# Eric-Canas/Homography.js

Measured on AMD Instinct MI355X. Metric: Mpixels/s warped (piecewise-affine, 4K RGBA), higher is better.
Workload: dtype u8 pixels / f64 coordinates

## Files before the change

### homography.js_amd/csrc/hg_api_piecewise.hip

```cpp
#include "hg_ctx.h"

extern "C" int hg_piecewise_set_mesh(hg_ctx *c, const float *src, int n_pts, const uint32_t *tris, int n_tris, int msx, int msy)
{
    HG_TRY(bind(c));
    if (!src || n_pts <= 0 || n_tris < 0 || (!tris && n_tris > 0)) return fail(c, HG_ERR_INVALID, "hg_piecewise_set_mesh: bad arguments");
    if (!coords_ok(src, (size_t)n_pts * 2))
        return fail(c, HG_ERR_INVALID, "hg_piecewise_set_mesh: a source coordinate is infinite or beyond 2^24 in magnitude");
    if (c->have_mesh && n_pts == c->n_pts && n_tris == c->n_tris && msx == c->min_src_x && msy == c->min_src_y &&
        std::memcmp(src, c->h_src.data(), sizeof(float) * 2 * (size_t)n_pts) == 0 &&
        (n_tris == 0 || std::memcmp(tris, c->h_tris.data(), sizeof(uint32_t) * 3 * (size_t)n_tris) == 0))
        return HG_OK;
    HG_TRY(hg_sync(c));
    HG_TRY(ensure(c, c->d_src, (size_t)n_pts * 2));
    HG_TRY(ensure(c, c->d_tris, (size_t)std::max(n_tris, 1) * 3));
    HIP_TRY(c, hipMemcpyAsync(c->d_src, src, sizeof(float) * 2 * n_pts, hipMemcpyHostToDevice, c->stream));
    if (n_tris > 0) HIP_TRY(c, hipMemcpyAsync(c->d_tris, tris, sizeof(uint32_t) * 3 * n_tris, hipMemcpyHostToDevice, c->stream));
    HIP_TRY(c, hipStreamSynchronize(c->stream));
    c->n_pts = n_pts; c->n_tris = n_tris; c->min_src_x = msx; c->min_src_y = msy;
    c->h_tris.assign(tris, tris + (size_t)3 * n_tris);
    c->h_src.assign(src, src + (size_t)2 * n_pts);
    c->fmap_valid = false;
    c->have_mesh = true;
    c->mesh_gen++; c->pw_epoch++;
    c->fwd_pw_tiles_disabled = false; c->fwd_pw_cap = 64;
// ... 407 lines not shown
    c->status_next = c->status_base + (size_t)((c->status_slot + 1) % (int)kStatusRing) * F;
    c->rows_clean = false;
    if (p.self) {
        c->pw_gen = c->pw_gen >= 0x7ffffff0 ? 1 : c->pw_gen + 1;
        launch_tri_setup(mesh_of(c), frames_of(c), c->stream);
    } else launch_tri_spans(mesh_of(c), frames_of(c), rl, c->stream);
    HIP_TRY(c, hipGetLastError());
    c->pw_setup_done = true;
    return HG_OK;
}

static SpanPlanKey span_key_of(const hg_ctx *c)
{
    const PwPlan &p = c->pw_plan;
    SpanPlanKey k;
    k.eligible = p.kernel == PwKernel::Rows && p.self && p.row_group == kRowGroup && c->n_imgs <= 1;
    k.W = c->W; k.H = c->H;
    if (c->pw_moving) { k.ms_lo_x = c->ms_lo_x; k.ms_hi_x = c->ms_hi_x; k.ms_lo_y = c->ms_lo_y; k.ms_hi_y = c->ms_hi_y; }
    else { k.ms_lo_x = k.ms_hi_x = c->min_src_x; k.ms_lo_y = k.ms_hi_y = c->min_src_y; }
    k.hi_bounds = p.no_hi_bounds ? 0 : 1;
    k.safe_spans = p.safe_spans; k.bands = p.bands ? 1 : 0; k.n_bands = p.n_bands;
    k.n_frames = (int)c->pw_frames.size(); k.max_h = c->pw_shape.max_h;
    return k;
}

static int span_cache_prepare(hg_ctx *c, SpanCacheDev *sc)
{
    *sc = SpanCacheDev();
    c->span_last = 0;
    if (c->opt_span_cache == 0) return HG_OK;
    const SpanPlanKey key = span_key_of(c);
    if (!key.eligible) return HG_OK;
    const PwShape &s = c->pw_shape;
    const uint64_t estimate = (uint64_t)s.groups * kRowGroup * (uint64_t)std::min(s.cover + 1, 63) * (kSpanRecWordsLong * 16);
    const bool force = c->opt_span_cache_mb < 0;
    const uint64_t budget = force ? (uint64_t)(-(int64_t)c->opt_span_cache_mb) << 10 : (uint64_t)c->opt_span_cache_mb << 20;
    const SpanCacheMode mode = span_cache_decide(c->span_state, c->pw_epoch, key, c->opt_span_cache, budget, estimate, force);
    if (mode == SpanCacheMode::Build) {
        const uint64_t bytes = std::min<uint64_t>(force ? budget : std::min(budget, estimate), ((uint64_t)1 << 36) - 16);
        const int gpf = (std::max(s.max_h, 1) + kRowGroup - 1) / kRowGroup;
        const size_t entries = 1 + (size_t)key.n_frames * gpf;
        HG_TRY(ensure(c, c->d_span_rec, (size_t)std::max<uint64_t>(bytes / 16, 1)));
        HG_TRY(ensure(c, c->d_span_dir, entries));
        HIP_TRY(c, hipMemsetAsync(c->d_span_dir, 0, sizeof(int4) * entries, c->stream));
        c->span_cap16 = (uint32_t)(bytes / 16); c->span_gpf = gpf;
        c->span_builds++;
    }
    span_cache_commit(c->span_state, c->pw_epoch, key, c->opt_span_cache, mode);
    if (mode == SpanCacheMode::Off) return HG_OK;
    if (mode == SpanCacheMode::Use) c->span_uses++;
    c->span_last = (int)mode;
    sc->dir = c->d_span_dir + 1; sc->rec = c->d_span_rec; sc->cursor = reinterpret_cast<unsigned long long *>(c->d_span_dir.p);
    sc->cap16 = c->span_cap16; sc->groups_per_frame = c->span_gpf; sc->mode = (int)mode;
    return HG_OK;
}

extern "C" int hg_span_cache_stats(hg_ctx *c, int64_t out[6])
{
    HG_TRY(bind(c));
    if (!out) return fail(c, HG_ERR_INVALID, "hg_span_cache_stats: out is NULL");
    out[0] = c->span_builds; out[1] = c->span_uses; out[2] = 0; out[3] = 0; out[4] = 0; out[5] = c->span_last;
    const SpanCacheState &st = c->span_state;
    if (!st.built || st.epoch != c->pw_epoch || !c->d_span_dir.cap || (size_t)st.key.n_frames != c->pw_frames.size()) return HG_OK;
    const size_t entries = 1 + (size_t)st.key.n_frames * c->span_gpf;
    std::vector<int4> dir(entries);
    HIP_TRY(c, hipStreamSynchronize(c->stream));
    HIP_TRY(c, hipMemcpy(dir.data(), c->d_span_dir, sizeof(int4) * entries, hipMemcpyDeviceToHost));
    for (size_t f = 0; f < c->pw_frames.size(); f++) {
        const FrameDesc &fd = c->pw_frames[f];
        if (fd.obj_w <= 0 || fd.obj_h <= 0) continue;
        for (int g = 0; g < (fd.obj_h + kRowGroup - 1) / kRowGroup; g++) {
            const int32_t state = dir[1 + f * (size_t)c->span_gpf + g].x;
// ... 364 lines not shown
```

### homography.js_amd/csrc/hg_dev.h

```cpp
#pragma once
#include "hg_kernels.h"
#include <cstdlib>
#include <type_traits>

namespace hg {

__device__ __forceinline__ void flag_frame(const PwFrames &fr, int f, int32_t bits)
{
    atomicOr(&fr.status[f], bits);
    if (fr.host_flag) __hip_atomic_store(fr.host_flag, 1, __ATOMIC_RELAXED, __HIP_MEMORY_SCOPE_SYSTEM);
}



extern "C" __device__ uint32_t hg_struct_load_u32(__amdgpu_buffer_rsrc_t rsrc, int vindex, int voffset, int soffset, int aux) __asm("llvm.amdgcn.struct.ptr.buffer.load.i32");

__device__ __forceinline__ bool frame_group(const PwFrames &fr, int xcd, int bi, int groups_per_xcd, int &f, int &g)
{
    if (fr.sub_groups > 0) {
        const int per_sub = fr.sub_groups * fr.n_frames, sb = bi / per_sub, rem = bi - sb * per_sub;
        f = rem / fr.sub_groups;
        g = ((sb << fr.xcc_log2) + xcd) * fr.sub_groups + (rem - f * fr.sub_groups);
        return g < (groups_per_xcd << fr.xcc_log2);
    }
    f = bi / groups_per_xcd;
    g = ((xcd + (fr.xcc_rotate ? f : 0)) & ((1 << fr.xcc_log2) - 1)) * groups_per_xcd + (bi - f * groups_per_xcd);
    return true;
}
inline int sub_groups_of(const PwFrames &fr, int groups_per_xcd) { return fr.sub_bands > 1 ? (groups_per_xcd + fr.sub_bands - 1) / fr.sub_bands : 0; }
inline int padded_groups(int groups_per_xcd, int sub_groups) { return sub_groups > 0 ? ((groups_per_xcd + sub_groups - 1) / sub_groups) * sub_groups : groups_per_xcd; }

struct HiBounds { uint32_t lox, rx, loy, ry; };
__host__ __device__ __forceinline__ bool hi_bounds_ok(int64_t ax, int64_t bx, int64_t ay, int64_t by)
{
    return ax >= 0 && ay >= 0 && bx < (1 << 20) && by < (1 << 20) && ax <= bx && ay <= by;
}
inline bool set_hi_bounds_ok(const PwMesh &mesh, const PwFrames &fr)
{
    if (!fr.min_src) return hi_bounds_ok(mesh.min_src_x, (int64_t)mesh.W + mesh.min_src_x, mesh.min_src_y, (int64_t)mesh.H + mesh.min_src_y);
    return hi_bounds_ok(fr.min_src_lo_x, (int64_t)mesh.W + fr.min_src_hi_x, fr.min_src_lo_y, (int64_t)mesh.H + fr.min_src_hi_y);
}
__device__ __forceinline__ HiBounds make_hi_bounds(double lox, double hix, double loy, double hiy)
{
    HiBounds b;
    b.lox = (uint32_t)__builtin_amdgcn_readfirstlane(__double2hiint(lox)); b.rx = (uint32_t)__builtin_amdgcn_readfirstlane(__double2hiint(hix)) - b.lox;
    b.loy = (uint32_t)__builtin_amdgcn_readfirstlane(__double2hiint(loy)); b.ry = (uint32_t)__builtin_amdgcn_readfirstlane(__double2hiint(hiy)) - b.loy;
    return b;
}
__device__ __forceinline__ bool hi_inb(const HiBounds &b, double hx, double hy)
{
    return (int)(((uint32_t)__double2hiint(hx) - b.lox) < b.rx) & (int)(((uint32_t)__double2hiint(hy) - b.loy) < b.ry);
}

__device__ __forceinline__ int round_inbounds(double x)
{
    double r = floor(x);
    if (x - r >= 0.5) r += 1.0;
    return (int)r;
}

__device__ __forceinline__ int64_t floordiv64(int64_t n, int64_t d)
{
    int64_t q = n / d;
    if ((n % d) < 0) --q;
    return q;
}

__device__ __forceinline__ uint32_t fetch_src(const uint32_t *__restrict__ img32, int64_t n_src_px, int W, int rx, int ry)
{
    const int64_t idx = (int64_t)ry * W + rx;
    return (idx >= 0 && idx < n_src_px) ? img32[idx] : 0u;
}

__device__ __forceinline__ void store_quad(uint32_t *__restrict__ orow, int cq, int W, bool vec_ok, const uint32_t px[4])
{
    if (vec_ok && cq + 3 < W) {
        *reinterpret_cast<uint4 *>(orow + cq) = make_uint4(px[0], px[1], px[2], px[3]);
    } else {
#pragma unroll
// ... 79 lines not shown

__device__ __forceinline__ uint32_t pw_pixel_bilinear(int tid_raw, int x, double y, MatCache &mc, const float *__restrict__ invm,
                                                      const uint32_t *__restrict__ img32, int W, int H,
                                                      double bx0, double bx1, double by0, double by1)
{
    const int t16 = (int)(int16_t)tid_raw;
    if (t16 < 0) return 0u;
    if (t16 != mc.id) {
        const float4 lo = *reinterpret_cast<const float4 *>(invm + (size_t)t16 * kInvStride);
        const float2 hi = *reinterpret_cast<const float2 *>(invm + (size_t)t16 * kInvStride + 4);
        mc.m[0] = lo.x; mc.m[1] = lo.y; mc.m[2] = lo.z; mc.m[3] = lo.w; mc.m[4] = hi.x; mc.m[5] = hi.y;
        mc.id = t16;
    }
    const double xd = (double)x;
    const double sx = (mc.m[0] * xd) + (mc.m[2] * y) + mc.m[4];
    const double sy = (mc.m[1] * xd) + (mc.m[3] * y) + mc.m[5];
    if (sx >= bx0 && sx < bx1 && sy >= by0 && sy < by1) return bilinear_fetch(img32, W, H, sx, sy);
    return 0u;
}

template <int S>
__device__ __forceinline__ uint32_t pw_pixel_mode(int tid_raw, int x, double y, MatCache &mc, const float *__restrict__ invm,
                                                  const uint32_t *__restrict__ img32, int64_t n_src_px, int W, int H,
                                                  double bx0, double bx1, double by0, double by1)
{
    if (S == 1) return pw_pixel_bilinear(tid_raw, x, y, mc, invm, img32, W, H, bx0, bx1, by0, by1);
    return pw_pixel(tid_raw, x, y, mc, invm, img32, n_src_px, W, H, bx0, bx1, by0, by1);
}

__device__ __forceinline__ uint32_t dlo(double v) { return (uint32_t)__double2loint(v); }
__device__ __forceinline__ double sgpr_f64(double v)
{
    return __hiloint2double(__builtin_amdgcn_readfirstlane(__double2hiint(v)), __builtin_amdgcn_readfirstlane(__double2loint(v)));
}

constexpr int kStoreNT = 2;
constexpr int kKeyShift = 14, kKeyOffMask = (1 << kKeyShift) - 1;

__device__ __forceinline__ void round_x8(double h[8], double r[8])
{
    const double M = 6755399441055744.0;
    asm(
        "s_setreg_imm32_b32 hwreg(HW_REG_MODE, 2, 2), 2\n\t"
        "v_add_f64 %0, %0, 0.5\n\t"  "v_add_f64 %1, %1, 0.5\n\t"  "v_add_f64 %2, %2, 0.5\n\t"  "v_add_f64 %3, %3, 0.5\n\t"
        "v_add_f64 %4, %4, 0.5\n\t"  "v_add_f64 %5, %5, 0.5\n\t"  "v_add_f64 %6, %6, 0.5\n\t"  "v_add_f64 %7, %7, 0.5\n\t"
        "v_add_f64 %8, %0, %16\n\t"  "v_add_f64 %9, %1, %16\n\t"  "v_add_f64 %10, %2, %16\n\t" "v_add_f64 %11, %3, %16\n\t"
        "v_add_f64 %12, %4, %16\n\t" "v_add_f64 %13, %5, %16\n\t" "v_add_f64 %14, %6, %16\n\t" "v_add_f64 %15, %7, %16\n\t"
        "s_setreg_imm32_b32 hwreg(HW_REG_MODE, 2, 2), 0"
        : "+v"(h[0]), "+v"(h[1]), "+v"(h[2]), "+v"(h[3]), "+v"(h[4]), "+v"(h[5]), "+v"(h[6]), "+v"(h[7]),
          "=&v"(r[0]), "=&v"(r[1]), "=&v"(r[2]), "=&v"(r[3]), "=&v"(r[4]), "=&v"(r[5]), "=&v"(r[6]), "=&v"(r[7])
        : "s"(M));
}

__device__ __forceinline__ void round_x4(double h[4], double r[4])
{
    const double M = 6755399441055744.0;
    asm volatile(
        "s_setreg_imm32_b32 hwreg(HW_REG_MODE, 2, 2), 2\n\t"
        "v_add_f64 %0, %0, 0.5\n\t" "v_add_f64 %1, %1, 0.5\n\t" "v_add_f64 %2, %2, 0.5\n\t" "v_add_f64 %3, %3, 0.5\n\t"
        "v_add_f64 %4, %0, %8\n\t"  "v_add_f64 %5, %1, %8\n\t"  "v_add_f64 %6, %2, %8\n\t"  "v_add_f64 %7, %3, %8\n\t"
        "s_setreg_imm32_b32 hwreg(HW_REG_MODE, 2, 2), 0"
        : "+v"(h[0]), "+v"(h[1]), "+v"(h[2]), "+v"(h[3]), "=&v"(r[0]), "=&v"(r[1]), "=&v"(r[2]), "=&v"(r[3])
        : "s"(M));
}

__device__ __forceinline__ void round_half_x4(const double v[4], int r[4])
// ... 38 lines not shown
        : [d0] "v"(d), [d1] "v"(d1), [d2] "v"(d2), [d3] "v"(d3), [len] "v"(len), [key] "v"(key)
        : "vcc");
}

__device__ __forceinline__ void span_max4s(int best[4], int d, int len, int key)
{
    const int d1 = d + 64, d2 = d + 128, d3 = d + 192;
    unsigned long long sv;
    asm volatile(
        "s_mov_b64 %[sv], exec\n\t"
        "v_cmpx_gt_u32_e32 vcc, %[len], %[d0]\n\t" "v_max_i32_e32 %[b0], %[key], %[b0]\n\t" "s_mov_b64 exec, %[sv]\n\t"
        "v_cmpx_gt_u32_e32 vcc, %[len], %[d1]\n\t" "v_max_i32_e32 %[b1], %[key], %[b1]\n\t" "s_mov_b64 exec, %[sv]\n\t"
        "v_cmpx_gt_u32_e32 vcc, %[len], %[d2]\n\t" "v_max_i32_e32 %[b2], %[key], %[b2]\n\t" "s_mov_b64 exec, %[sv]\n\t"
        "v_cmpx_gt_u32_e32 vcc, %[len], %[d3]\n\t" "v_max_i32_e32 %[b3], %[key], %[b3]\n\t" "s_mov_b64 exec, %[sv]"
        : [b0] "+v"(best[0]), [b1] "+v"(best[1]), [b2] "+v"(best[2]), [b3] "+v"(best[3]), [sv] "=&s"(sv)
        : [d0] "v"(d), [d1] "v"(d1), [d2] "v"(d2), [d3] "v"(d3), [len] "s"(len), [key] "s"(key)
        : "vcc");
}

__device__ __forceinline__ void span_max4d(int best[4], int d0, int d1, int d2, int d3, int len, int key)
{
    unsigned long long sv;
    asm volatile(
        "s_mov_b64 %[sv], exec\n\t"
        "v_cmpx_lt_u32_e32 vcc, %[d0], %[len]\n\t" "v_max_i32_e32 %[b0], %[b0], %[key]\n\t" "s_mov_b64 exec, %[sv]\n\t"
        "v_cmpx_lt_u32_e32 vcc, %[d1], %[len]\n\t" "v_max_i32_e32 %[b1], %[b1], %[key]\n\t" "s_mov_b64 exec, %[sv]\n\t"
        "v_cmpx_lt_u32_e32 vcc, %[d2], %[len]\n\t" "v_max_i32_e32 %[b2], %[b2], %[key]\n\t" "s_mov_b64 exec, %[sv]\n\t"
        "v_cmpx_lt_u32_e32 vcc, %[d3], %[len]\n\t" "v_max_i32_e32 %[b3], %[b3], %[key]\n\t" "s_mov_b64 exec, %[sv]"
        : [b0] "+v"(best[0]), [b1] "+v"(best[1]), [b2] "+v"(best[2]), [b3] "+v"(best[3]), [sv] "=&s"(sv)
        : [d0] "v"(d0), [d1] "v"(d1), [d2] "v"(d2), [d3] "v"(d3), [len] "v"(len), [key] "v"(key)
        : "vcc");
}

}

#include "hg_spans.h"
```

### homography.js_amd/csrc/hg_k_piecewise.hip

```cpp
#include "hg_dev.h"
#include <type_traits>

namespace hg {

constexpr int kBandMax = 2048;

__device__ __forceinline__ bool tri_setup_one(const PwMesh &mesh, const PwFrames &fr, int f, int t, const FrameDesc &fd, TriRange &tr)
{
    float d[6], inv[6];
    Seg seg[3];
    tri_solve(mesh, fr, f, t, true, d, inv, seg);
    const size_t ft = (size_t)f * mesh.n_tris + t;
    const bool one_fma = affine_fusable(inv, coord_bits(fd.x_off, fd.obj_w), coord_bits(fd.y_off, fd.obj_h));

    tri_rows_tight(d[1], d[3], d[5], tr.y_min, tr.y_end);
    tr.a = 0; tr.b = 0;
    const bool too_tall = (tr.y_end - (int64_t)tr.y_min) > (1 << 24);
    {
        int64_t y_first = tr.y_min, y_stop = tr.y_end;
        if (fd.obj_w > 0 && fd.obj_h > 0) clamp_rows(y_first, y_stop, fd.y_off, fd.obj_w, (int64_t)fd.obj_w * fd.obj_h);
        else y_stop = y_first;
        if (y_stop < y_first) y_stop = y_first;
        tr.y_min = (int32_t)y_first; tr.y_end = (int32_t)y_stop;
    }
// ... 244 lines not shown
    if (r0 >= fd.obj_h || fd.obj_w <= 0) return;

    __shared__ __align__(16) double s_m[CAP * 6];
    __shared__ int s_lo[CAP], s_hi[CAP], s_len[CAP], s_key[CAP];
    constexpr int RG = kRowGroup;
    static_assert(CAP >= 64 * RG, "packed mode gives each of the RG rows a 64-slot block");
    constexpr int KS = CAP * 48 <= (1 << kKeyShift) ? kKeyShift : kKeyShift + 1, KMASK = (1 << KS) - 1;
    static_assert(CAP * 48 <= (1 << KS) && KS <= 15, "record offsets must fit below the 15-bit id");
    constexpr int KADDR = KMASK & ~15;

    const int W = fd.obj_w;
    const int lane = threadIdx.x & 63;
    const int wave = __builtin_amdgcn_readfirstlane((int)(threadIdx.x >> 6));
    const int nwin_row = (W + 255) >> 8;
    const int w_lo = 0, nwin = nwin_row;
    const int nrows = min(rows_per_group, fd.obj_h - r0);

    constexpr int kCandCap = SELF ? 256 : 1;
    __shared__ int s_cnt[RG], s_ncand;
    __shared__ int s_cand_tn[kCandCap], s_cand_y[kCandCap];
    int cnts[RG], cmax = 0;
    if (!SELF) {
        const int32_t *cntp = rl.cnt + (size_t)f * rl.row_stride + r0;
#pragma unroll
        for (int j = 0; j < RG; j++) { cnts[j] = j < nrows ? cntp[j] : 0; cmax = max(cmax, cnts[j]); }
        if (cmax > rl.cap || cmax > CAP - 1) {
            if (threadIdx.x == 0) flag_frame(fr, f, FRAME_LDS_OVERFLOW);
            return;
        }
    }
    const bool packed = SELF ? rows_per_group == RG : (rows_per_group == RG && __builtin_amdgcn_readfirstlane(cmax) <= 63);

    const __amdgpu_buffer_rsrc_t src = __builtin_amdgcn_make_buffer_rsrc(const_cast<uint8_t *>(frame_img(mesh, f)), 4, mesh.W * mesh.H, 0x00020000);
    const double bx_lo = sgpr_f64((double)ms.x + 0.5), bx_hi = sgpr_f64((double)mesh.W + (double)ms.x + 0.5);
    const double by_lo = sgpr_f64((double)ms.y + 0.5), by_hi = sgpr_f64((double)mesh.H + (double)ms.y + 0.5);
    const HiBounds hb = make_hi_bounds((double)ms.x + 0.5, (double)mesh.W + (double)ms.x + 0.5,
                                       (double)ms.y + 0.5, (double)mesh.H + (double)ms.y + 0.5);
    const bool flag_spans = fr.safe_spans != 0;
    const bool one_fma = SELF != 0 && fr.two_round && __builtin_amdgcn_readfirstlane(fr.two_round[f]) != fr.gen;
    auto unsafe_bit = [&](double m0, double m2y, double m4, double m1, double m3y, double m5, int lo, int hi) -> int {
        return span_unsafe<HIB>(flag_spans, hb, bx_lo, bx_hi, by_lo, by_hi, fd.x_off, m0, m2y, m4, m1, m3y, m5, lo, hi);
    };

    const float *__restrict__ ginv = fr.inv + (size_t)f * mesh.n_tris * kInvStride;
    auto load_row = [&](int row, int cnt, int base, int nan_slot, int t0, int step) {
        const double y = (double)(r0 + row + fd.y_off);
        const size_t e0 = ((size_t)f * rl.row_stride + r0 + row) * rl.cap;
        for (int i = t0; i < cnt; i += step) {
            uint32_t lh, id;
            double m0, m1, m2, m3, m4, m5;
            if (COMPACT) {
                const uint2 a = static_cast<const uint2 *>(rl.ent)[e0 + i];
                lh = a.x; id = a.y;
                const float4 ma = *reinterpret_cast<const float4 *>(ginv + (size_t)id * kInvStride);
                const float2 mb = *reinterpret_cast<const float2 *>(ginv + (size_t)id * kInvStride + 4);
                m0 = (double)ma.x; m1 = (double)ma.y; m2 = (double)ma.z; m3 = (double)ma.w; m4 = (double)mb.x; m5 = (double)mb.y;
            } else {
                const uint4 a = static_cast<const uint4 *>(rl.ent)[2 * (e0 + i)], b = static_cast<const uint4 *>(rl.ent)[2 * (e0 + i) + 1];
                lh = a.x; id = a.y;
                m0 = (double)__uint_as_float(a.z); m1 = (double)__uint_as_float(a.w); m2 = (double)__uint_as_float(b.x);
                m3 = (double)__uint_as_float(b.y); m4 = (double)__uint_as_float(b.z); m5 = (double)__uint_as_float(b.w);
            }
            const int elo = (int)(lh & 0xffffu), ehi = (int)(lh >> 16);
            s_lo[base + i] = elo; s_hi[base + i] = ehi; s_len[base + i] = ehi - elo;
            s_key[base + i] = ((int)id << KS) | ((base + i) * 48) | unsafe_bit(m0, m2 * y, m4, m1, m3 * y, m5, elo, ehi);
            double2 *mrec = reinterpret_cast<double2 *>(s_m + (base + i) * 6);
            mrec[0] = make_double2(m0, m2 * y);
            mrec[1] = make_double2(m1, m3 * y);
            mrec[2] = make_double2(m4, m5);
        }
// ... 36 lines not shown
                if (r < r0) r = r0;
                for (; r < r0 + nrows; r++) {
                    const int rb = r * W;
                    if (rb >= fin) break;
                    const int lo = max(k - rb, 0), hi = min(fin - rb, W);
                    if (lo >= hi) continue;
                    const int row = r - r0;
                    const int slot = atomicAdd(&s_cnt[row], 1);
                    if (slot >= capr) continue;
                    const int at = (packed ? row * 64 : 0) + slot;
                    const double yr = (double)(r + fd.y_off);
                    const double m2y = (double)ma.z * yr, m3y = (double)ma.w * yr;
                    s_lo[at] = lo; s_hi[at] = hi; s_len[at] = hi - lo;
                    s_key[at] = (t << KS) | (at * 48) | unsafe_bit((double)ma.x, m2y, (double)mb.x, (double)ma.y, m3y, (double)mb.y, lo, hi);
                    double2 *mrec = reinterpret_cast<double2 *>(s_m + at * 6);
                    if (one_fma) {
                        mrec[0] = make_double2((double)ma.x, m2y + (double)mb.x);
                        mrec[1] = make_double2((double)ma.y, m3y + (double)mb.y);
                    } else {
                        mrec[0] = make_double2((double)ma.x, m2y);
                        mrec[1] = make_double2((double)ma.y, m3y);
                        mrec[2] = make_double2((double)mb.x, (double)mb.y);
                    }
                }
            }
        }
        __syncthreads();
        bool ok = true;
#pragma unroll
        for (int j = 0; j < RG; j++) { cnts[j] = j < nrows ? s_cnt[j] : 0; ok = ok && cnts[j] <= capr; }
        return ok;
    };

    auto do_row = [&](int row, int cnt, int base, int nan_slot, int w0, int wstep) {
        const int nan_key = (int)0x80000000u | ((base + nan_slot) * 48) | 1;
        const int r = r0 + row;
        const int64_t row_px = (int64_t)r * W;
        const __amdgpu_buffer_rsrc_t dst = __builtin_amdgcn_make_buffer_rsrc(out + fd.out_off + row_px * 4, 0, W * 4, 0x00020000);
        const bool vec_zero = ((W & 3) == 0) && (((fd.out_off + (uint64_t)row_px * 4) & 15) == 0);
        typedef uint32_t v4u __attribute__((ext_vector_type(4)));
        const v4u zero4 = { 0u, 0u, 0u, 0u };
        const bool in_regs = cnt <= 64;
        int lo_r = 0x7fffffff, hi_r = 0, key_r = 0;
        if (in_regs && lane < cnt) { lo_r = s_lo[base + lane]; hi_r = s_hi[base + lane]; key_r = s_key[base + lane]; }
        for (int wb = w0; wb < nwin; wb += wstep * PH) {
            uint32_t px[PH][4];
            bool empty[PH];
#pragma unroll
            for (int p = 0; p < PH; p++) {
                const int w = wb + p * wstep;
                if (w >= nwin) break;
                const int c0 = w << 8, cq = c0 + lane;
                int best[4];
#pragma unroll
                for (int k = 0; k < 4; k++) best[k] = nan_key;
                unsigned long long any = 0ull;
                if (in_regs) {
                    unsigned long long mask = __ballot(lo_r < c0 + 256 && hi_r > c0);
                    any = mask;
                    while (mask) {
                        const int bit = __ffsll((long long)mask) - 1;
                        mask &= mask - 1;
                        const int lo = __builtin_amdgcn_readlane(lo_r, bit);
                        span_max4s(best, cq - lo, __builtin_amdgcn_readlane(hi_r, bit) - lo, __builtin_amdgcn_readlane(key_r, bit));
                    }
                } else for (int j = 0; j < cnt; j += 64) {
                    const int idx = j + lane;
                    int lo = 0x7fffffff, hi = 0;
                    if (idx < cnt) { lo = s_lo[base + idx]; hi = s_hi[base + idx]; }
                    unsigned long long mask = __ballot(lo < c0 + 256 && hi > c0);
                    any |= mask;
                    while (mask) {
                        const int bit = __ffsll((long long)mask) - 1;
                        mask &= mask - 1;
                        const int slot = base + j + bit;
                        const int d = cq - s_lo[slot];
                        span_max4(best, d, s_len[slot], s_key[slot]);
                    }
                }
                empty[p] = any == 0;
                if (empty[p]) px[p][0] = px[p][1] = px[p][2] = px[p][3] = 0u;
                else {
                    const double xd0 = (double)(cq + fd.x_off);
                    constexpr int STEP = PH == 1 ? 4 : 2;
                    auto coords = [&](auto n_tag, int k0, double *v) {
                        constexpr int N = decltype(n_tag)::value;
                        if constexpr (SELF == 0) {
#pragma unroll
                            for (int k = 0; k < N; k++) {
                                const double2 *mrec = reinterpret_cast<const double2 *>(reinterpret_cast<const char *>(s_m) + (best[k0 + k] & KADDR));
                                const double2 ra = mrec[0], rb = mrec[1], rc = mrec[2];
                                const double xd = xd0 + (double)((k0 + k) * 64);
                                v[2 * k] = fma(ra.x, xd, ra.y) + rc.x; v[2 * k + 1] = fma(rb.x, xd, rb.y) + rc.y;
                            }
                        } else {
#pragma unroll
                            for (int k = 0; k < N; k++) {
                                const double2 *mrec = reinterpret_cast<const double2 *>(reinterpret_cast<const char *>(s_m) + (best[k0 + k] & KADDR));
                                const double2 ra = mrec[0], rb = mrec[1];
                                const double xd = xd0 + (double)((k0 + k) * 64);
                                v[2 * k] = fma(ra.x, xd, ra.y); v[2 * k + 1] = fma(rb.x, xd, rb.y);
                            }
                            if (!one_fma) {
#pragma unroll
                                for (int k = 0; k < N; k++) {
                                    const double2 rc = reinterpret_cast<const double2 *>(reinterpret_cast<const char *>(s_m) + (best[k0 + k] & KADDR))[2];
                                    v[2 * k] += rc.x; v[2 * k + 1] += rc.y;
                                }
                            }
                        }
                    };
                    typedef std::integral_constant<int, 2> two_t;
                    typedef std::integral_constant<int, STEP> step_t;
                    const bool safe = flag_spans && __ballot(((best[0] | best[1] | best[2] | best[3]) & 1) != 0) == 0ull;
                    if (safe) {
#pragma unroll
                        for (int kk = 0; kk < 4; kk += 2) {
                            if (kk == 2 && c0 + 128 >= W) { px[p][2] = px[p][3] = 0u; continue; }
                            double v[4];
                            int r[4];
                            coords(two_t{}, kk, v);
                            round_half_x4(v, r);
#pragma unroll
                            for (int k = kk; k < kk + 2; k++)
                                px[p][k] = hg_struct_load_u32(src, __mul24(r[2 * (k - kk) + 1], mesh.W) + r[2 * (k - kk)], 0, 0, 0);
                        }
                    } else
#pragma unroll
                    for (int kk = 0; kk < 4; kk += STEP) {
                        if (STEP == 2 && kk == 2 && c0 + 128 >= W) { px[p][2] = px[p][3] = 0u; continue; }
                        double h[2 * STEP], rd[2 * STEP];
                        coords(step_t{}, kk, h);
                        if constexpr (STEP == 4) round_x8(h, rd); else round_x4(h, rd);
#pragma unroll
                        for (int k = kk; k < kk + STEP; k++) {
                            const int q = 2 * (k - kk);
                            const bool inb = HIB ? hi_inb(hb, h[q], h[q + 1])
                                                 : (bool)((int)(h[q] >= bx_lo) & (int)(h[q] < bx_hi) & (int)(h[q + 1] >= by_lo) & (int)(h[q + 1] < by_hi));
                            const int o = __mul24((int)dlo(rd[q + 1]), mesh.W) + (int)dlo(rd[q]);
                            px[p][k] = hg_struct_load_u32(src, inb ? o : -1, 0, 0, 0);
                        }
                    }
                }
                if (MAP) {
#pragma unroll
                    for (int k = 0; k < 4; k++)
                        if (cq + k * 64 < W) map_out[fd.map_off + row_px + cq + k * 64] = best[k] < 0 ? (int16_t)-1 : (int16_t)(best[k] >> KS);
                }
            }
#pragma unroll
            for (int p = 0; p < PH; p++) {
                const int w = wb + p * wstep;
                if (w >= nwin) break;
                const int cq = (w << 8) + lane;
                if (empty[p] && vec_zero) {
                    __builtin_amdgcn_raw_buffer_store_b128(zero4, dst, ((w << 8) + lane * 4) * 4, 0, kStoreNT);
                } else {
#pragma unroll
                    for (int k = 0; k < 4; k++) __builtin_amdgcn_raw_buffer_store_b32(px[p][k], dst, (cq + k * 64) * 4, 0, kStoreNT);
                }
            }
        }
    };

    if (SELF) {
        bool have = false;
        if constexpr (SELF >= 2) {
            typedef uint32_t v4u __attribute__((ext_vector_type(4)));
            auto dir_at = [&]() -> size_t { return (size_t)__builtin_amdgcn_readfirstlane(f) * sc.groups_per_frame + __builtin_amdgcn_readfirstlane(gi); };
            auto rec_words = [&]() -> int { return one_fma ? kSpanRecWordsFma : kSpanRecWordsLong; };
            if constexpr (SELF == 3) {
                const size_t di = dir_at();
                const int recw = rec_words(), crow = wave;
                const int4 e = sc.dir[di];
                const int state = __builtin_amdgcn_readfirstlane(e.x);
                if (packed && state == SPAN_DIR_OVERFLOWED) {
                    if (threadIdx.x == 0) flag_frame(fr, f, FRAME_LDS_OVERFLOW);
                    return;
                }
                if (packed && state == SPAN_DIR_VALID && __builtin_amdgcn_readfirstlane(e.w) == recw) {
                    const uint32_t off16 = (uint32_t)__builtin_amdgcn_readfirstlane(e.y), counts = (uint32_t)__builtin_amdgcn_readfirstlane(e.z);
                    if (lane < 3) reinterpret_cast<double2 *>(s_m + (crow * 64 + 63) * 6)[lane] = make_double2(NAN, NAN);
                    int before = 0;
#pragma unroll
                    for (int j = 0; j < RG; j++) { cnts[j] = span_count(counts, j); before += j < crow ? cnts[j] : 0; }
                    if (lane < span_count(counts, crow)) {
                        const v4u *p = reinterpret_cast<const v4u *>(sc.rec) + off16 + (size_t)(before + lane) * recw;
                        const v4u a = p[0], b = p[1];
                        const int at = crow * 64 + lane, lo = span_lo(a.x), hi = span_hi(a.x);
                        s_lo[at] = lo; s_hi[at] = hi; s_len[at] = hi - lo;
                        s_key[at] = (span_id(a.y) << KS) | (at * 48) | span_unsafe_bit(a.y);
                        double2 *mrec = reinterpret_cast<double2 *>(s_m + at * 6);
                        mrec[0] = make_double2((double)__uint_as_float(a.z), __hiloint2double((int)b.y, (int)b.x));
                        mrec[1] = make_double2((double)__uint_as_float(a.w), __hiloint2double((int)b.w, (int)b.z));
                        if (!one_fma) {
                            const v4u c = p[2];
                            mrec[2] = make_double2((double)__uint_as_float(c.x), (double)__uint_as_float(c.y));
                        }
                    }
                    have = true;
                }
            }
            if (!have) {
                const bool ok = self_prologue();
                if (SELF == 2 && packed) {
                    const size_t di = dir_at();
                    const int recw = rec_words(), crow = wave;
                    if (threadIdx.x == 0) {
                        SpanDirEnt d{ok ? SPAN_DIR_NOT_CACHED : SPAN_DIR_OVERFLOWED, 0u, 0u, 0u};
                        if (ok) {
                            const unsigned long long need = (unsigned long long)(cnts[0] + cnts[1] + cnts[2] + cnts[3]) * recw;
                            const unsigned long long at16 = atomicAdd(sc.cursor, need);
                            if (at16 + need <= sc.cap16) { d.state = SPAN_DIR_VALID; d.off16 = (uint32_t)at16; d.counts = span_pack_counts(cnts[0], cnts[1], cnts[2], cnts[3]); }
                        }
                        sc.dir[di] = make_int4(d.state, (int)d.off16, (int)d.counts, recw);
                        s_cand_tn[0] = d.state; s_cand_y[0] = (int)d.off16;
                    }
                    __syncthreads();
                    if (s_cand_tn[0] == SPAN_DIR_VALID) {
                        const uint32_t off16 = (uint32_t)s_cand_y[0];
                        int before = 0, mine = 0;
#pragma unroll
                        for (int j = 0; j < RG; j++) { before += j < crow ? cnts[j] : 0; mine += j == crow ? cnts[j] : 0; }
                        if (lane < mine) {
                            v4u *p = reinterpret_cast<v4u *>(sc.rec) + off16 + (size_t)(before + lane) * recw;
                            const int at = crow * 64 + lane, key = s_key[at];
                            const double2 *mrec = reinterpret_cast<const double2 *>(s_m + at * 6);
                            const double2 ra = mrec[0], rb = mrec[1];
                            const v4u a = { span_pack_lo_hi(s_lo[at], s_hi[at]), span_pack_id(key >> KS, key & 1), __float_as_uint((float)ra.x), __float_as_uint((float)rb.x) };
                            const v4u b = { (uint32_t)__double2loint(ra.y), (uint32_t)__double2hiint(ra.y), (uint32_t)__double2loint(rb.y), (uint32_t)__double2hiint(rb.y) };
                            __builtin_nontemporal_store(a, p); __builtin_nontemporal_store(b, p + 1);
                            if (!one_fma) {
                                const double2 rc = mrec[2];
                                const v4u c = { __float_as_uint((float)rc.x), __float_as_uint((float)rc.y), 0u, 0u };
                                __builtin_nontemporal_store(c, p + 2);
                            }
                        }
                    }
                }
                if (!ok) {
                    if (threadIdx.x == 0) flag_frame(fr, f, FRAME_LDS_OVERFLOW);
                    return;
                }
            }
        } else
        if (!self_prologue()) {
            if (threadIdx.x == 0) flag_frame(fr, f, FRAME_LDS_OVERFLOW);
            return;
        }
        const int row = packed ? wave : 0;
        int cnt_row = 0;
#pragma unroll
        for (int j = 0; j < RG; j++) cnt_row += cnts[j] * (row == j);
        const int cnt = __builtin_amdgcn_readfirstlane(cnt_row);
        if (row < nrows) do_row(row, cnt, packed ? wave * 64 : 0, packed ? 63 : CAP - 1, w_lo + (packed ? 0 : wave), packed ? 1 : nwaves);
        return;
    }
    const int npass = packed ? 1 : nrows;
    for (int pass = 0; pass < npass; pass++) {
        const int row = packed ? wave : pass;
        const int cnt = __builtin_amdgcn_readfirstlane(cnts[0] * (row == 0) + cnts[1] * (row == 1) + cnts[2] * (row == 2) + cnts[3] * (row == 3));
        const int base = packed ? wave * 64 : 0, nan_slot = packed ? 63 : CAP - 1;
        load_row(row, cnt, base, nan_slot, packed ? lane : (int)threadIdx.x, packed ? 64 : nthreads);
        __syncthreads();
        if (row < nrows) do_row(row, cnt, base, nan_slot, w_lo + (packed ? 0 : wave), packed ? 1 : nwaves);
        if (!packed) __syncthreads();
    }
}

template <int CAP, bool MAP, int PH = 1, bool COMPACT = false, bool HIB = false, int SELF = 0>
__global__ __launch_bounds__(256) void k_pw_rows(PwMesh mesh, PwFrames fr, RowLists rl, uint8_t *__restrict__ out, int16_t *__restrict__ map_out,
                                                 int groups_per_xcd, int rows_per_group, int32_t *__restrict__ status_next)
{
    pw_rows_body<CAP, MAP, PH, COMPACT, HIB, SELF>(mesh, fr, rl, out, map_out, groups_per_xcd, rows_per_group, status_next, SpanCacheDev());
}

template <int PH, bool HIB, int SELF>
__global__ __launch_bounds__(256) void k_pw_rows_cached(PwMesh mesh, PwFrames fr, RowLists rl, uint8_t *__restrict__ out, int groups_per_xcd, int rows_per_group,
                                                        int32_t *__restrict__ status_next, SpanCacheDev sc)
{
    static_assert(SELF == 2 || SELF == 3, "build or use");
    pw_rows_body<kRowSpanCapFast, false, PH, false, HIB, SELF>(mesh, fr, rl, out, nullptr, groups_per_xcd, rows_per_group, status_next, sc);
}

template <int CAP, bool MAP, int PH = 1, bool COMPACT = false, bool HIB = false, int SELF = 0>
__global__ __launch_bounds__(256) __attribute__((amdgpu_num_sgpr(80))) void k_pw_rows_s80(PwMesh mesh, PwFrames fr, RowLists rl, uint8_t *__restrict__ out,
                                                 int16_t *__restrict__ map_out, int groups_per_xcd, int rows_per_group, int32_t *__restrict__ status_next)
{
    pw_rows_body<CAP, MAP, PH, COMPACT, HIB, SELF>(mesh, fr, rl, out, map_out, groups_per_xcd, rows_per_group, status_next, SpanCacheDev());
}

__global__ __launch_bounds__(256) void k_upload(UploadSegs sg)
{
#pragma unroll
    for (int k = 0; k < 3; k++) {
        uint2 *__restrict__ dst = static_cast<uint2 *>(sg.dst[k]);
        const uint2 *__restrict__ src = static_cast<const uint2 *>(sg.src[k]);
        for (size_t i = (size_t)blockIdx.x * 256 + threadIdx.x; i < sg.n8[k]; i += (size_t)gridDim.x * 256) dst[i] = src[i];
// ... 118 lines not shown
```

### homography.js_amd/csrc/hg_kernels.h

```cpp
#pragma once
#include <hip/hip_runtime.h>
#include <stdint.h>
#include "hg_math.h"
#include "hg_span_cache.h"
#include "hg_remap_records.h"

namespace hg {

struct FrameDesc {
    int32_t x_off, y_off, obj_w, obj_h;
    uint64_t out_off;
    uint64_t map_off;
};

struct TriRange { int32_t y_min, y_end, a, b; };

enum : int32_t {
    FRAME_OK = 0,
    FRAME_IRREGULAR = 1,
    FRAME_LDS_OVERFLOW = 2
};

constexpr int kRowSpanCap = 1024;
constexpr int kRowSpanCapFast = 256;
constexpr int kRowSpanCapDense = 512;
constexpr int kRowGroup = 4;
constexpr int kInvStride = 8;

struct PwMesh {
    const float *src_pts;
    const uint32_t *tris;
    int32_t n_pts, n_tris;
    int32_t min_src_x, min_src_y;
    const uint8_t *img;
    int32_t W, H;
    int32_t n_imgs;
    uint64_t img_stride;
// ... 175 lines not shown
```

Measured before the change: 1.189 million.

## Cache span rows as sorted non-overlapping runs to replace per-pixel winner search

When the span cache is built, each row's overlapping triangle spans are resolved into a sorted list of disjoint runs, each tagged with its owning triangle, a gap flag and an unsafe flag. On cache use, the row kernel finds the owning record for each pixel by counting run starts with ballots and compare/add-carry, in place of the key-max search over overlapping spans. The goal is to cut per-window selection work in the cached replay path. It adds build-time O(n²) candidate work, a larger worst-case cache allocation and inline asm that pins values to registers, and it depends on runs fitting within 64 per row.

```diff
diff --git a/homography.js_amd/csrc/hg_api_piecewise.hip b/homography.js_amd/csrc/hg_api_piecewise.hip
--- a/homography.js_amd/csrc/hg_api_piecewise.hip
+++ b/homography.js_amd/csrc/hg_api_piecewise.hip
@@ -463,12 +463,14 @@
     const SpanPlanKey key = span_key_of(c);
     if (!key.eligible) return HG_OK;
     const PwShape &s = c->pw_shape;
-    const uint64_t estimate = (uint64_t)s.groups * kRowGroup * (uint64_t)std::min(s.cover + 1, 63) * (kSpanRecWordsLong * 16);
+    const uint64_t spans_row = (uint64_t)std::min(s.cover + 1, kRunSpanCap), runs_row = std::min<uint64_t>(2 * spans_row + 1, kRunCap);
+    const uint64_t estimate = (uint64_t)s.groups * kRowGroup * spans_row * (kSpanRecWordsLong * 16);
+    const uint64_t worst = (uint64_t)s.groups * kRowGroup * runs_row * (kSpanRecWordsLong * 16);
     const bool force = c->opt_span_cache_mb < 0;
     const uint64_t budget = force ? (uint64_t)(-(int64_t)c->opt_span_cache_mb) << 10 : (uint64_t)c->opt_span_cache_mb << 20;
     const SpanCacheMode mode = span_cache_decide(c->span_state, c->pw_epoch, key, c->opt_span_cache, budget, estimate, force);
     if (mode == SpanCacheMode::Build) {
-        const uint64_t bytes = std::min<uint64_t>(force ? budget : std::min(budget, estimate), ((uint64_t)1 << 36) - 16);
+        const uint64_t bytes = std::min<uint64_t>(force ? budget : std::min(budget, worst), ((uint64_t)1 << 36) - 16);
         const int gpf = (std::max(s.max_h, 1) + kRowGroup - 1) / kRowGroup;
         const size_t entries = 1 + (size_t)key.n_frames * gpf;
         HG_TRY(ensure(c, c->d_span_rec, (size_t)std::max<uint64_t>(bytes / 16, 1)));
diff --git a/homography.js_amd/csrc/hg_dev.h b/homography.js_amd/csrc/hg_dev.h
--- a/homography.js_amd/csrc/hg_dev.h
+++ b/homography.js_amd/csrc/hg_dev.h
@@ -45,6 +45,17 @@
     HiBounds b;
     b.lox = (uint32_t)__builtin_amdgcn_readfirstlane(__double2hiint(lox)); b.rx = (uint32_t)__builtin_amdgcn_readfirstlane(__double2hiint(hix)) - b.lox;
     b.loy = (uint32_t)__builtin_amdgcn_readfirstlane(__double2hiint(loy)); b.ry = (uint32_t)__builtin_amdgcn_readfirstlane(__double2hiint(hiy)) - b.loy;
+    return b;
+}
+__device__ __forceinline__ uint32_t pin_u32(uint32_t v)
+{
+    asm volatile("" : "+v"(v));
+    return (uint32_t)__builtin_amdgcn_readfirstlane((int)v);
+}
+template <bool PIN>
+__device__ __forceinline__ HiBounds pin_hi_bounds(HiBounds b)
+{
+    if constexpr (PIN) { b.lox = pin_u32(b.lox); b.rx = pin_u32(b.rx); b.loy = pin_u32(b.loy); b.ry = pin_u32(b.ry); }
     return b;
 }
 __device__ __forceinline__ bool hi_inb(const HiBounds &b, double hx, double hy)
@@ -190,6 +201,15 @@
 __device__ __forceinline__ double sgpr_f64(double v)
 {
     return __hiloint2double(__builtin_amdgcn_readfirstlane(__double2hiint(v)), __builtin_amdgcn_readfirstlane(__double2loint(v)));
+}
+
+template <bool PIN>
+__device__ __forceinline__ double pin_f64(double v)
+{
+    if constexpr (PIN) {
+        return __hiloint2double((int)pin_u32((uint32_t)__double2hiint(v)), (int)pin_u32((uint32_t)__double2loint(v)));
+    }
+    return v;
 }
 
 constexpr int kStoreNT = 2;
@@ -294,6 +314,23 @@
         : "vcc");
 }
 
+__device__ __forceinline__ void run_count4(int idx[4], int q, int s)
+{
+    const int s1 = s - 64, s2 = s - 128, s3 = s - 192;
+    unsigned long long c0, c1, c2, c3;
+    asm volatile("v_cmp_le_i32_e64 %[c0], %[s0], %[q]\n\t" "v_cmp_le_i32_e64 %[c1], %[s1], %[q]\n\t"
+        "v_cmp_le_i32_e64 %[c2], %[s2], %[q]\n\t" "v_cmp_le_i32_e64 %[c3], %[s3], %[q]\n\t"
+        "v_addc_co_u32_e64 %[i0], %[c0], 0, %[i0], %[c0]\n\t" "v_addc_co_u32_e64 %[i1], %[c1], 0, %[i1], %[c1]\n\t"
+        "v_addc_co_u32_e64 %[i2], %[c2], 0, %[i2], %[c2]\n\t" "v_addc_co_u32_e64 %[i3], %[c3], 0, %[i3], %[c3]"
+        : [i0] "+v"(idx[0]), [i1] "+v"(idx[1]), [i2] "+v"(idx[2]), [i3] "+v"(idx[3]), [c0] "=&s"(c0), [c1] "=&s"(c1), [c2] "=&s"(c2), [c3] "=&s"(c3)
+        : [q] "v"(q), [s0] "s"(s), [s1] "s"(s1), [s2] "s"(s2), [s3] "s"(s3));
+}
+__device__ __forceinline__ void run_off4(int off[4], const int idx[4], int base)
+{
+#pragma unroll
+    for (int k = 0; k < 4; k++) asm volatile("v_mad_u32_u24 %0, %1, 48, %2" : "=v"(off[k]) : "v"(idx[k]), "s"(base));
+}
+
 }
 
 #include "hg_spans.h"
diff --git a/homography.js_amd/csrc/hg_k_piecewise.hip b/homography.js_amd/csrc/hg_k_piecewise.hip
--- a/homography.js_amd/csrc/hg_k_piecewise.hip
+++ b/homography.js_amd/csrc/hg_k_piecewise.hip
@@ -300,10 +300,10 @@
     const bool packed = SELF ? rows_per_group == RG : (rows_per_group == RG && __builtin_amdgcn_readfirstlane(cmax) <= 63);
 
     const __amdgpu_buffer_rsrc_t src = __builtin_amdgcn_make_buffer_rsrc(const_cast<uint8_t *>(frame_img(mesh, f)), 4, mesh.W * mesh.H, 0x00020000);
-    const double bx_lo = sgpr_f64((double)ms.x + 0.5), bx_hi = sgpr_f64((double)mesh.W + (double)ms.x + 0.5);
-    const double by_lo = sgpr_f64((double)ms.y + 0.5), by_hi = sgpr_f64((double)mesh.H + (double)ms.y + 0.5);
-    const HiBounds hb = make_hi_bounds((double)ms.x + 0.5, (double)mesh.W + (double)ms.x + 0.5,
-                                       (double)ms.y + 0.5, (double)mesh.H + (double)ms.y + 0.5);
+    const double bx_lo = pin_f64<SELF == 3>(sgpr_f64((double)ms.x + 0.5)), bx_hi = pin_f64<SELF == 3>(sgpr_f64((double)mesh.W + (double)ms.x + 0.5));
+    const double by_lo = pin_f64<SELF == 3>(sgpr_f64((double)ms.y + 0.5)), by_hi = pin_f64<SELF == 3>(sgpr_f64((double)mesh.H + (double)ms.y + 0.5));
+    const HiBounds hb = pin_hi_bounds<SELF == 3>(make_hi_bounds((double)ms.x + 0.5, (double)mesh.W + (double)ms.x + 0.5,
+                                                                (double)ms.y + 0.5, (double)mesh.H + (double)ms.y + 0.5));
     const bool flag_spans = fr.safe_spans != 0;
     const bool one_fma = SELF != 0 && fr.two_round && __builtin_amdgcn_readfirstlane(fr.two_round[f]) != fr.gen;
     auto unsafe_bit = [&](double m0, double m2y, double m4, double m1, double m3y, double m5, int lo, int hi) -> int {
@@ -406,7 +406,11 @@
         return ok;
     };
 
-    auto do_row = [&](int row, int cnt, int base, int nan_slot, int w0, int wstep) {
+    bool runs = false;
+    int run_start_r = 0x7fffffff;
+    unsigned long long run_unsafe_m = 0ull, run_gap_m = 0ull;
+
+    auto do_row = [&](auto run_tag, int row, int cnt, int base, int nan_slot, int w0, int wstep) {
         const int nan_key = (int)0x80000000u | ((base + nan_slot) * 48) | 1;
         const int r = r0 + row;
         const int64_t row_px = (int64_t)r * W;
@@ -415,8 +419,10 @@
         typedef uint32_t v4u __attribute__((ext_vector_type(4)));
         const v4u zero4 = { 0u, 0u, 0u, 0u };
         const bool in_regs = cnt <= 64;
+        constexpr bool run_form = decltype(run_tag)::value;
         int lo_r = 0x7fffffff, hi_r = 0, key_r = 0;
-        if (in_regs && lane < cnt) { lo_r = s_lo[base + lane]; hi_r = s_hi[base + lane]; key_r = s_key[base + lane]; }
+        if (!run_form && in_regs && lane < cnt) { lo_r = s_lo[base + lane]; hi_r = s_hi[base + lane]; key_r = s_key[base + lane]; }
+        if constexpr (run_form) lo_r = run_start_r;
         for (int wb = w0; wb < nwin; wb += wstep * PH) {
             uint32_t px[PH][4];
             bool empty[PH];
@@ -429,6 +435,23 @@
 #pragma unroll
                 for (int k = 0; k < 4; k++) best[k] = nan_key;
                 unsigned long long any = 0ull;
+                bool safe_w = false;
+                if constexpr (run_form) {
+                    const unsigned long long m_le = __ballot(lo_r <= c0), interior = __ballot(lo_r < c0 + 256) & ~m_le;
+                    const int first = __popcll(m_le) - 1;
+                    const int first48 = (base + first) * 48;
+                    if (interior) {
+                        int idx[4] = { 0, 0, 0, 0 };
+                        for (unsigned long long mask = interior; mask; mask &= mask - 1)
+                            run_count4(idx, cq, __builtin_amdgcn_readlane(lo_r, __ffsll((long long)mask) - 1));
+                        run_off4(best, idx, first48);
+                    } else {
+#pragma unroll
+                        for (int k = 0; k < 4; k++) best[k] = first48;
+                    }
+                    any = run_window_empty(run_gap_m, first, interior) ? 0ull : 1ull;
+                    safe_w = flag_spans && run_window_safe(run_unsafe_m, run_range(first, interior));
+                } else
                 if (in_regs) {
                     unsigned long long mask = __ballot(lo_r < c0 + 256 && hi_r > c0);
                     any = mask;
@@ -470,7 +493,7 @@
                         } else {
 #pragma unroll
                             for (int k = 0; k < N; k++) {
-                                const double2 *mrec = reinterpret_cast<const double2 *>(reinterpret_cast<const char *>(s_m) + (best[k0 + k] & KADDR));
+                                const double2 *mrec = reinterpret_cast<const double2 *>(reinterpret_cast<const char *>(s_m) + (run_form ? best[k0 + k] : (best[k0 + k] & KADDR)));
                                 const double2 ra = mrec[0], rb = mrec[1];
                                 const double xd = xd0 + (double)((k0 + k) * 64);
                                 v[2 * k] = fma(ra.x, xd, ra.y); v[2 * k + 1] = fma(rb.x, xd, rb.y);
@@ -478,7 +501,7 @@
                             if (!one_fma) {
 #pragma unroll
                                 for (int k = 0; k < N; k++) {
-                                    const double2 rc = reinterpret_cast<const double2 *>(reinterpret_cast<const char *>(s_m) + (best[k0 + k] & KADDR))[2];
+                                    const double2 rc = reinterpret_cast<const double2 *>(reinterpret_cast<const char *>(s_m) + (run_form ? best[k0 + k] : (best[k0 + k] & KADDR)))[2];
                                     v[2 * k] += rc.x; v[2 * k + 1] += rc.y;
                                 }
                             }
@@ -486,7 +509,7 @@
                     };
                     typedef std::integral_constant<int, 2> two_t;
                     typedef std::integral_constant<int, STEP> step_t;
-                    const bool safe = flag_spans && __ballot(((best[0] | best[1] | best[2] | best[3]) & 1) != 0) == 0ull;
+                    const bool safe = run_form ? safe_w : flag_spans && __ballot(((best[0] | best[1] | best[2] | best[3]) & 1) != 0) == 0ull;
                     if (safe) {
 #pragma unroll
                         for (int kk = 0; kk < 4; kk += 2) {
@@ -528,6 +551,12 @@
                 if (w >= nwin) break;
                 const int cq = (w << 8) + lane;
                 if (empty[p] && vec_zero) {
+                    if constexpr (run_form) {
+                        uint32_t z, o;
+                        asm volatile("v_mov_b32 %0, 0\n\tv_lshl_add_u32 %1, %2, 4, %3" : "=&v"(z), "=v"(o) : "v"(lane), "s"(w << 10));
+                        const v4u z4 = { z, z, z, z };
+                        __builtin_amdgcn_raw_buffer_store_b128(z4, dst, (int)o, 0, kStoreNT);
+                    } else
                     __builtin_amdgcn_raw_buffer_store_b128(zero4, dst, ((w << 8) + lane * 4) * 4, 0, kStoreNT);
                 } else {
 #pragma unroll
@@ -554,16 +583,15 @@
                 }
                 if (packed && state == SPAN_DIR_VALID && __builtin_amdgcn_readfirstlane(e.w) == recw) {
                     const uint32_t off16 = (uint32_t)__builtin_amdgcn_readfirstlane(e.y), counts = (uint32_t)__builtin_amdgcn_readfirstlane(e.z);
-                    if (lane < 3) reinterpret_cast<double2 *>(s_m + (crow * 64 + 63) * 6)[lane] = make_double2(NAN, NAN);
                     int before = 0;
 #pragma unroll
                     for (int j = 0; j < RG; j++) { cnts[j] = span_count(counts, j); before += j < crow ? cnts[j] : 0; }
+                    bool r_unsafe = false, r_gap = false;
                     if (lane < span_count(counts, crow)) {
                         const v4u *p = reinterpret_cast<const v4u *>(sc.rec) + off16 + (size_t)(before + lane) * recw;
                         const v4u a = p[0], b = p[1];
-                        const int at = crow * 64 + lane, lo = span_lo(a.x), hi = span_hi(a.x);
-                        s_lo[at] = lo; s_hi[at] = hi; s_len[at] = hi - lo;
-                        s_key[at] = (span_id(a.y) << KS) | (at * 48) | span_unsafe_bit(a.y);
+                        const int at = crow * 64 + lane;
+                        run_start_r = run_start(a.x); r_gap = run_gap(a.x) != 0; r_unsafe = span_unsafe_bit(a.y) != 0;
                         double2 *mrec = reinterpret_cast<double2 *>(s_m + at * 6);
                         mrec[0] = make_double2((double)__uint_as_float(a.z), __hiloint2double((int)b.y, (int)b.x));
                         mrec[1] = make_double2((double)__uint_as_float(a.w), __hiloint2double((int)b.w, (int)b.z));
@@ -572,6 +600,8 @@
                             mrec[2] = make_double2((double)__uint_as_float(c.x), (double)__uint_as_float(c.y));
                         }
                     }
+                    run_unsafe_m = __ballot(r_unsafe); run_gap_m = __ballot(r_gap);
+                    runs = true;
                     have = true;
                 }
             }
@@ -580,12 +610,24 @@
                 if (SELF == 2 && packed) {
                     const size_t di = dir_at();
                     const int recw = rec_words(), crow = wave;
+                    __shared__ uint32_t s_rcand[RG * kRunCands], s_runs[RG * kRunCap];
+                    __shared__ int s_nruns[RG];
+                    int cnt_mine = 0;
+#pragma unroll
+                    for (int j = 0; j < RG; j++) cnt_mine += j == crow ? cnts[j] : 0;
+                    if (ok) run_candidates(s_lo + crow * 64, s_hi + crow * 64, s_key + crow * 64, cnt_mine, W, KS, lane, s_rcand + crow * kRunCands);
+                    __syncthreads();
+                    if (ok) {
+                        const int nr = run_place(s_rcand + crow * kRunCands, cnt_mine, lane, s_runs + crow * kRunCap);
+                        if (lane == 0) s_nruns[crow] = crow < nrows ? nr : 0;
+                    }
+                    __syncthreads();
                     if (threadIdx.x == 0) {
                         SpanDirEnt d{ok ? SPAN_DIR_NOT_CACHED : SPAN_DIR_OVERFLOWED, 0u, 0u, 0u};
-                        if (ok) {
-                            const unsigned long long need = (unsigned long long)(cnts[0] + cnts[1] + cnts[2] + cnts[3]) * recw;
+                        if (ok && max(max(s_nruns[0], s_nruns[1]), max(s_nruns[2], s_nruns[3])) <= kRunCap) {
+                            const unsigned long long need = (unsigned long long)(s_nruns[0] + s_nruns[1] + s_nruns[2] + s_nruns[3]) * recw;
                             const unsigned long long at16 = atomicAdd(sc.cursor, need);
-                            if (at16 + need <= sc.cap16) { d.state = SPAN_DIR_VALID; d.off16 = (uint32_t)at16; d.counts = span_pack_counts(cnts[0], cnts[1], cnts[2], cnts[3]); }
+                            if (at16 + need <= sc.cap16) { d.state = SPAN_DIR_VALID; d.off16 = (uint32_t)at16; d.counts = span_pack_counts(s_nruns[0], s_nruns[1], s_nruns[2], s_nruns[3]); }
                         }
                         sc.dir[di] = make_int4(d.state, (int)d.off16, (int)d.counts, recw);
                         s_cand_tn[0] = d.state; s_cand_y[0] = (int)d.off16;
@@ -595,13 +637,14 @@
                         const uint32_t off16 = (uint32_t)s_cand_y[0];
                         int before = 0, mine = 0;
 #pragma unroll
-                        for (int j = 0; j < RG; j++) { before += j < crow ? cnts[j] : 0; mine += j == crow ? cnts[j] : 0; }
+                        for (int j = 0; j < RG; j++) { before += j < crow ? s_nruns[j] : 0; mine += j == crow ? s_nruns[j] : 0; }
                         if (lane < mine) {
                             v4u *p = reinterpret_cast<v4u *>(sc.rec) + off16 + (size_t)(before + lane) * recw;
-                            const int at = crow * 64 + lane, key = s_key[at];
+                            const uint32_t e = s_runs[crow * kRunCap + lane];
+                            const int gap = run_ent_gap(e), at = crow * 64 + (gap ? 63 : run_ent_slot(e)), key = s_key[crow * 64 + run_ent_slot(e)];
                             const double2 *mrec = reinterpret_cast<const double2 *>(s_m + at * 6);
                             const double2 ra = mrec[0], rb = mrec[1];
-                            const v4u a = { span_pack_lo_hi(s_lo[at], s_hi[at]), span_pack_id(key >> KS, key & 1), __float_as_uint((float)ra.x), __float_as_uint((float)rb.x) };
+                            const v4u a = { run_pack_start(run_ent_start(e), gap), span_pack_id(gap ? 0 : key >> KS, run_ent_unsafe(e)), __float_as_uint((float)ra.x), __float_as_uint((float)rb.x) };
                             const v4u b = { (uint32_t)__double2loint(ra.y), (uint32_t)__double2hiint(ra.y), (uint32_t)__double2loint(rb.y), (uint32_t)__double2hiint(rb.y) };
                             __builtin_nontemporal_store(a, p); __builtin_nontemporal_store(b, p + 1);
                             if (!one_fma) {
@@ -627,7 +670,10 @@
 #pragma unroll
         for (int j = 0; j < RG; j++) cnt_row += cnts[j] * (row == j);
         const int cnt = __builtin_amdgcn_readfirstlane(cnt_row);
-        if (row < nrows) do_row(row, cnt, packed ? wave * 64 : 0, packed ? 63 : CAP - 1, w_lo + (packed ? 0 : wave), packed ? 1 : nwaves);
+        if (row < nrows) {
+            if constexpr (SELF == 3) { if (runs) { do_row(std::true_type{}, row, cnt, wave * 64, 63, w_lo, 1); return; } }
+            do_row(std::false_type{}, row, cnt, packed ? wave * 64 : 0, packed ? 63 : CAP - 1, w_lo + (packed ? 0 : wave), packed ? 1 : nwaves);
+        }
         return;
     }
     const int npass = packed ? 1 : nrows;
@@ -637,7 +683,7 @@
         const int base = packed ? wave * 64 : 0, nan_slot = packed ? 63 : CAP - 1;
         load_row(row, cnt, base, nan_slot, packed ? lane : (int)threadIdx.x, packed ? 64 : nthreads);
         __syncthreads();
-        if (row < nrows) do_row(row, cnt, base, nan_slot, w_lo + (packed ? 0 : wave), packed ? 1 : nwaves);
+        if (row < nrows) do_row(std::false_type{}, row, cnt, base, nan_slot, w_lo + (packed ? 0 : wave), packed ? 1 : nwaves);
         if (!packed) __syncthreads();
     }
 }
diff --git a/homography.js_amd/csrc/hg_kernels.h b/homography.js_amd/csrc/hg_kernels.h
--- a/homography.js_amd/csrc/hg_kernels.h
+++ b/homography.js_amd/csrc/hg_kernels.h
@@ -3,6 +3,7 @@
 #include <stdint.h>
 #include "hg_math.h"
 #include "hg_span_cache.h"
+#include "hg_span_runs.h"
 #include "hg_remap_records.h"
 
 namespace hg {
diff --git a/homography.js_amd/csrc/hg_span_runs.h b/homography.js_amd/csrc/hg_span_runs.h
--- /dev/null
+++ b/homography.js_amd/csrc/hg_span_runs.h
@@ -0,0 +1,105 @@
+#pragma once
+#include "hg_span_cache.h"
+
+namespace hg {
+
+constexpr int kRunCap = 64;
+constexpr int kRunSpanCap = 63;
+constexpr int kRunCands = 2 * 64;
+
+HG_SC_FN uint32_t run_pack_start(int start, int gap) { return (uint32_t)start | ((uint32_t)(gap & 1) << 16); }
+HG_SC_FN int run_start(uint32_t w) { return (int)(w & 0xffffu); }
+HG_SC_FN int run_gap(uint32_t w) { return (int)((w >> 16) & 1u); }
+
+HG_SC_FN uint32_t run_ent(int start, int slot, int gap, int unsafe) { return (uint32_t)start | ((uint32_t)slot << 16) | ((uint32_t)gap << 22) | ((uint32_t)unsafe << 23); }
+HG_SC_FN int run_ent_start(uint32_t e) { return (int)(e & 0xffffu); }
+HG_SC_FN int run_ent_slot(uint32_t e) { return (int)((e >> 16) & 63u); }
+HG_SC_FN int run_ent_gap(uint32_t e) { return (int)((e >> 22) & 1u); }
+HG_SC_FN int run_ent_unsafe(uint32_t e) { return (int)((e >> 23) & 1u); }
+constexpr uint32_t kRunEntStarts = 1u << 24, kRunEntMask = kRunEntStarts - 1;
+
+HG_SC_FN void run_winners(const int *lo, const int *hi, const int *key, int cnt, int x, int *at, int *before)
+{
+    int a = -1, ak = 0, b = -1, bk = 0;
+    for (int i = 0; i < cnt; i++) {
+        const int l = lo[i], h = hi[i], k = key[i];
+        if (l <= x && x < h && (a < 0 || k > ak)) { a = i; ak = k; }
+        if (l < x && x <= h && (b < 0 || k > bk)) { b = i; bk = k; }
+    }
+    *at = a; *before = b;
+}
+
+HG_SC_FN bool run_cand_pos(const int *lo, const int *hi, int cnt, int W, int c, int *pos)
+{
+    const int i = c >> 1;
+    if (i < cnt) { *pos = (c & 1) ? hi[i] : lo[i]; return *pos < W; }
+    *pos = 0;
+    return c == 2 * 63;
+}
+
+HG_SC_FN void run_candidates(const int *lo, const int *hi, const int *key, int cnt, int W, int ks, int lane, uint32_t *cand)
+{
+    for (int b = 0; b < 2; b++) {
+        const int c = 2 * lane + b;
+        int pos;
+        uint32_t e = 0;
+        if (run_cand_pos(lo, hi, cnt, W, c, &pos)) {
+            int wa, wb;
+            run_winners(lo, hi, key, cnt, pos, &wa, &wb);
+            const int ida = wa < 0 ? -1 : key[wa] >> ks;
+            const int idb = pos == 0 ? -2 : wb < 0 ? -1 : key[wb] >> ks;
+            if (ida != idb) {
+                bool dup = false;
+                const int c_end = c < 2 * cnt ? c : 2 * cnt;
+                for (int c2 = 0; c2 < c_end && !dup; c2++) {
+                    int p2;
+                    dup = run_cand_pos(lo, hi, cnt, W, c2, &p2) && p2 == pos;
+                }
+                if (!dup) {
+                    int unsafe = wa < 0 ? 1 : 0;
+                    for (int i = 0; i < cnt; i++) unsafe |= ((key[i] >> ks) == ida) ? (key[i] & 1) : 0;
+                    e = run_ent(pos, wa < 0 ? 0 : wa, wa < 0 ? 1 : 0, unsafe) | kRunEntStarts;
+                }
+            }
+        }
+        cand[c] = e;
+    }
+}
+
+HG_SC_FN int run_place(const uint32_t *cand, int cnt, int lane, uint32_t *runs)
+{
+    const uint32_t zero = cand[2 * 63];
+    int n = (zero & kRunEntStarts) ? 1 : 0;
+    for (int c = 0; c < 2 * cnt; c++) n += (cand[c] & kRunEntStarts) ? 1 : 0;
+    if (n > kRunCap) return n;
+    for (int b = 0; b < 2; b++) {
+        const uint32_t e = cand[2 * lane + b];
+        if (!(e & kRunEntStarts)) continue;
+        int rank = (2 * lane + b != 2 * 63 && (zero & kRunEntStarts) && run_ent_start(e) > 0) ? 1 : 0;
+        for (int c = 0; c < 2 * cnt; c++) rank += ((cand[c] & kRunEntStarts) && run_ent_start(cand[c]) < run_ent_start(e)) ? 1 : 0;
+        runs[rank] = e & kRunEntMask;
+    }
+    return n;
+}
+
+HG_SC_FN void run_window(const int *start, int nruns, int c0, int *first, uint64_t *interior)
+{
+    uint64_t le = 0, lt = 0;
+    for (int i = 0; i < nruns; i++) {
+        le |= (uint64_t)(start[i] <= c0) << i;
+        lt |= (uint64_t)(start[i] < c0 + 256) << i;
+    }
+    *first = __builtin_popcountll(le) - 1;
+    *interior = lt & ~le;
+}
+HG_SC_FN int run_index(const int *start, int first, uint64_t interior, int x)
+{
+    int idx = first;
+    for (uint64_t m = interior; m; m &= m - 1) idx += x >= start[__builtin_ctzll(m)] ? 1 : 0;
+    return idx;
+}
+HG_SC_FN uint64_t run_range(int first, uint64_t interior) { return interior | ((uint64_t)1 << first); }
+HG_SC_FN bool run_window_safe(uint64_t unsafe_mask, uint64_t range) { return (unsafe_mask & range) == 0; }
+HG_SC_FN bool run_window_empty(uint64_t gap_mask, int first, uint64_t interior) { return interior == 0 && ((gap_mask >> first) & 1) != 0; }
+
+}
```

New measurement: 1.258 million (median of 6 runs). 1.06x the previous value.
